# KarelPeeters/kZero

Measured on AMD Instinct MI355X. Metric: self-play NN evals/sec (node), Chess 20x256 ResNet b=256, 1/2/4/8 GPU, higher is better.
Workload: dtype f16; 1 GPU; chess-20x256 attention head, executor batch 256; engines_per_gpu=1, parallelism=dp1 (no collective)

## Files before the change

kzero_amd/csrc/kz_tower.hip:

```cpp
#include <cstdlib>
#include <type_traits>
#include <vector>

#include "kz_kernels.hpp"
#include "kz_launch.hpp"

namespace kz {

typedef _Float16 h16;
typedef h16 h16x8 __attribute__((ext_vector_type(8)));
typedef h16 h16x4 __attribute__((ext_vector_type(4)));
typedef float f32x4 __attribute__((ext_vector_type(4)));

namespace {

#include "kz_decode_dev.hpp"
#include "kz_encode_dev.hpp"

constexpr int C = 256;
constexpr int RS = C * 2 + 16;
constexpr int URS = 3 * C * 2 + 16;
constexpr int KSTEPS = 72;
constexpr int HEAD_KSTEPS = 5 * 8;
constexpr int POLICY = 1880, LOGIT_LD = 96;
constexpr int TOWER_PF_MAX = 8;

struct TowerDev {
    const h16 *x0;
    const uint4 *w_stem, *w_tower;
    const float *bias, *post_scale, *post_shift;
    h16 *y;
    int cin_p, batch, depth;
    PackedBoards in;
    const float *sh_w0, *sh_b0, *sh_w1, *sh_b1, *sh_w2, *sh_b2;
    const int32_t *att_idx;
    float *scalars, *policy;
    int *nonfinite_flag;
    int epoch;
    DecodeDev dec;
};

template <int I, int N, class F>
__device__ __forceinline__ void static_for(F &&f) {
    if constexpr (I < N) {
        f(std::integral_constant<int, I>{});
        static_for<I + 1, N>(f);
    }
}

template <int NB>
struct Layout {
    static constexpr int M = NB * 64;
    static constexpr int MT = M / 16;
    static constexpr bool LINE_TILES = NB == 2;
    static constexpr int BPAD = LINE_TILES ? 128 : 0;
    static constexpr int BOARD = 64 * RS + BPAD;
    static constexpr int TS = LINE_TILES ? 8 * RS : 16 * RS;
    static constexpr int IMG = NB * BOARD;
    static constexpr int X_OFF = 0;
    static constexpr int Y_OFF = IMG;
    static constexpr int Z_OFF = 2 * IMG;
    static_assert(Z_OFF % 256 == 0, "zero rows keep the slot pattern of the image rows");
    static constexpr int S_OFF = Z_OFF + 16 * RS;
    static constexpr int TOWER_BYTES = S_OFF + M * 64;
    static constexpr int U_OFF = Z_OFF;
    static constexpr int ACT_OFF = U_OFF + 16 * URS;
    static constexpr int HID_OFF = ACT_OFF + NB * 256 * 4;
    static constexpr int HEADS_BYTES = HID_OFF + NB * 32 * 4;
    static constexpr int LOG_OFF = Y_OFF;
    static constexpr int BYTES = TOWER_BYTES > HEADS_BYTES ? TOWER_BYTES : HEADS_BYTES;
    static_assert(NB * 64 * LOGIT_LD * 4 <= IMG, "logits fit the Y region");
    static constexpr int row_off(int b, int p) { return b * BOARD + p * RS; }
    static_assert(BYTES <= 160 * 1024, "LDS budget");
};

constexpr int SG_VALU = 0x2, SG_SALU = 0x4, SG_MFMA = 0x8, SG_VMEM_READ = 0x20, SG_DS_READ = 0x100;

template <int NB, bool HEADS, int PF, bool WIDE = false, bool PREV = false>
__global__ __launch_bounds__(256, 1) void kz_tower_resident(TowerDev a) {
    using L = Layout<NB>;
    constexpr int M = L::M, MT = L::MT;
    static_assert(PF <= TOWER_PF_MAX, "the refills past the end of the stream must land in its padding");
    extern __shared__ __attribute__((aligned(16))) unsigned char lds[];

    const int tid = threadIdx.x;
    const int wave = __builtin_amdgcn_readfirstlane(tid >> 6);
    const int lane = tid & 63;
    const int fr = lane & 15, kq = lane >> 4;
    const int board0 = blockIdx.x * NB;
    const int layers = 2 * a.depth;
    const int total_ksteps = layers * KSTEPS + (HEADS ? HEAD_KSTEPS : 0);
    const int bias_rows = layers + (HEADS ? 5 : 0);

    const uint4 *wp = a.w_tower + wave * 256 + lane;
    auto wload_prev = [&](int gk, int nt) __attribute__((always_inline)) { return wp[(size_t)gk * 1024 + nt * 64]; };
    typedef const __attribute__((address_space(1))) unsigned char *gptr;
    gptr wk = (gptr)a.w_tower + wave * 4096;
    const unsigned wlane = lane * 16;
    auto wload = [&](gptr k, int nt) __attribute__((always_inline)) {
        typedef unsigned u32x4 __attribute__((ext_vector_type(4)));
        return __builtin_bit_cast(uint4, *reinterpret_cast<const __attribute__((address_space(1))) u32x4 *>(k + wlane + nt * 1024));
    };
    uint4 wreg[PF][4];
#pragma unroll
    for (int s = 0; s < PF; s++) {
        const int g = s < total_ksteps ? s : total_ksteps - 1;
#pragma unroll
        for (int nt = 0; nt < 4; nt++) wreg[s][nt] = PREV ? wload_prev(g, nt) : wload(wk + s * 16384, nt);
    }
    wk += PF * 16384;
    int g = 0;
    auto ring_take = [&](int stage, h16x8 (&af)[4]) __attribute__((always_inline)) {
#pragma unroll
        for (int nt = 0; nt < 4; nt++) af[nt] = *reinterpret_cast<const h16x8 *>(&wreg[stage][nt]);
#ifndef KZ_TW_NO_WLOAD
        if constexpr (PREV) {
            const int gn = g + PF < total_ksteps ? g + PF : total_ksteps - 1;
#pragma unroll
            for (int nt = 0; nt < 4; nt++) wreg[stage][nt] = wload_prev(gn, nt);
        } else {
#pragma unroll
            for (int nt = 0; nt < 4; nt++) wreg[stage][nt] = wload(wk, nt);
        }
#endif
        wk += 16384;
        if constexpr (!PREV) asm("" : "+s"(wk));
    };

    const int sc = WIDE ? a.cin_p >> 5 : 1;
    const int stem_off = WIDE ? L::Y_OFF : L::S_OFF, srow = 64 * sc, spieces = 4 * sc;
    for (int id = tid; id < 16 * RS / 16; id += 256)
        *reinterpret_cast<uint4 *>(lds + L::Z_OFF + id * 16) = make_uint4(0, 0, 0, 0);
    for (int id = tid; id < M * spieces; id += 256) {
        const int row = WIDE ? id / spieces : id >> 2, c = id - row * spieces;
        const int board = board0 + (row >> 6);
        uint4 v = make_uint4(0, 0, 0, 0);
        if (board < a.batch) {
            if (a.in.bits) {
                h16x8 e;
#pragma unroll
                for (int j = 0; j < 8; j++) e[j] = (h16)encoded_plane(a.in, board, c * 8 + j, row & 63, 64);
                v = *reinterpret_cast<const uint4 *>(&e);
            } else {
                v = *reinterpret_cast<const uint4 *>(a.x0 + ((size_t)board0 * 64 + row) * a.cin_p + c * 8);
            }
        }
        *reinterpret_cast<uint4 *>(lds + stem_off + row * srow + c * 16) = v;
    }
    __syncthreads();

    f32x4 acc[4][MT];
    f32x4 bias_next[4];
    auto fetch_bias = [&](int row) __attribute__((always_inline)) {
        const int l = row <= bias_rows ? row : bias_rows;
#pragma unroll
        for (int nt = 0; nt < 4; nt++)
            bias_next[nt] = *reinterpret_cast<const f32x4 *>(a.bias + l * C + wave * 64 + nt * 16 + kq * 4);
    };
    auto init_acc = [&]() __attribute__((always_inline)) {
#pragma unroll
        for (int nt = 0; nt < 4; nt++)
#pragma unroll
            for (int mt = 0; mt < MT; mt++) acc[nt][mt] = bias_next[nt];
    };
    f32x4 post_s[4], post_t[4];
#pragma unroll
    for (int nt = 0; nt < 4; nt++) {
        post_s[nt] = f32x4{1.f, 1.f, 1.f, 1.f};
        post_t[nt] = f32x4{0.f, 0.f, 0.f, 0.f};
    }

    auto relu4 = [](f32x4 v) {
        typedef int i32x4 __attribute__((ext_vector_type(4)));
        i32x4 b = __builtin_bit_cast(i32x4, v);
#pragma unroll
        for (int j = 0; j < 4; j++) b[j] = b[j] > 0 ? b[j] : 0;
        return __builtin_bit_cast(f32x4, b);
    };
    auto to_h4 = [](f32x4 v) { return h16x4{(h16)v[0], (h16)v[1], (h16)v[2], (h16)v[3]}; };

    const int lane_row = L::LINE_TILES ? (fr >> 3) * L::BOARD + (fr & 7) * RS : fr * RS;
    const int epi_base = lane_row + (wave * 64 + kq * 4) * 2;
    auto epilogue = [&](int dst_off, auto relu, auto residual, auto post) __attribute__((always_inline)) {
#pragma unroll
        for (int nt = 0; nt < 4; nt++) {
            h16x4 rx[MT];
            if constexpr (decltype(residual)::value) {
#pragma unroll
                for (int mt = 0; mt < MT; mt++)
                    rx[mt] = *reinterpret_cast<const h16x4 *>(lds + L::X_OFF + epi_base + mt * L::TS + nt * 32);
            }
#pragma unroll
            for (int mt = 0; mt < MT; mt++) {
                const int off = epi_base + mt * L::TS + nt * 32;
                f32x4 v = acc[nt][mt];
                if constexpr (decltype(relu)::value) v = relu4(v);
                if constexpr (decltype(residual)::value) {
#pragma unroll
                    for (int j = 0; j < 4; j++) v[j] += (float)rx[mt][j];
                }
                if constexpr (decltype(post)::value) v = v * post_s[nt] + post_t[nt];
                *reinterpret_cast<h16x4 *>(lds + dst_off + off) = to_h4(v);
            }
        }
    };
    constexpr std::true_type YES{};
    constexpr std::false_type NO{};

    const bool x_is0 = (lane & 7) == 0, x_is7 = (lane & 7) == 7, yo_is0 = (lane & 8) == 0, yo_is1 = !yo_is0;
    auto tap_ok = [&](int mt, int dy, int dx) __attribute__((always_inline)) {
        const bool kill_x = (dx < 0 && x_is0) || (dx > 0 && x_is7);
        if constexpr (L::LINE_TILES) return !(kill_x || (dy < 0 && mt == 0) || (dy > 0 && mt == MT - 1));
        else return !(kill_x || ((mt & 3) == 0 && dy < 0 && yo_is0) || ((mt & 3) == 3 && dy > 0 && yo_is1));
    };

    fetch_bias(0);
    init_acc();
    fetch_bias(1);
    for (int ks = 0; ks < 9 * sc; ks++) {
        const int tap = WIDE ? ks / sc : ks, chunk = ks - tap * sc;
        const int dy = tap / 3 - 1, dx = tap % 3 - 1;
        h16x8 af[4];
#pragma unroll
        for (int nt = 0; nt < 4; nt++) {
            const uint4 t = a.w_stem[((ks * 4 + wave) * 4 + nt) * 64 + lane];
            af[nt] = *reinterpret_cast<const h16x8 *>(&t);
        }
#pragma unroll
        for (int mt = 0; mt < MT; mt++) {
            const bool ok = tap_ok(mt, dy, dx);
            const int p = L::LINE_TILES ? (fr >> 3) * 64 + mt * 8 + (fr & 7) : mt * 16 + fr;
            const int off = ok ? stem_off + (p + dy * 8 + dx) * srow + chunk * 64 + kq * 16 : L::Z_OFF + kq * 16;
            const h16x8 bf = *reinterpret_cast<const h16x8 *>(lds + off);
#pragma unroll
            for (int nt = 0; nt < 4; nt++)
                acc[nt][mt] = __builtin_amdgcn_mfma_f32_16x16x32_f16(af[nt], bf, acc[nt][mt], 0, 0, 0);
        }
    }
    epilogue(L::X_OFF, NO, NO, NO);
    __syncthreads();

    const int kq_off = 256 * (kq & 1) + 128 * (kq >> 1);
    const int frag_base = lane_row + kq_off;
    auto tap_rows = [&](int dy, int dx, int src_off, int (&T)[MT]) __attribute__((always_inline)) {
        const int shifted = frag_base + src_off + (dy * 8 + dx) * RS;
        const int zrow = L::Z_OFF + ((fr + dy * 8 + dx) & 15) * RS + kq_off;
        const int zrow_odd = L::LINE_TILES ? L::Z_OFF + ((fr + dy * 8 + dx + 8) & 15) * RS + kq_off : zrow;
        if constexpr (PREV) {
#pragma unroll
            for (int mt = 0; mt < MT; mt++) T[mt] = tap_ok(mt, dy, dx) ? shifted + mt * L::TS : ((mt & 1) ? zrow_odd : zrow);
        } else {
            int z0 = zrow, z1 = zrow_odd;
            asm("" : "+v"(z0), "+v"(z1));
            const bool kill_x = ((dx < 0) & x_is0) | ((dx > 0) & x_is7);
#pragma unroll
            for (int mt = 0; mt < MT; mt++) {
                bool kill = kill_x;
                if constexpr (!L::LINE_TILES) kill = kill_x | (((mt & 3) == 0) & (dy < 0) & yo_is0) | (((mt & 3) == 3) & (dy > 0) & yo_is1);
                T[mt] = kill ? ((mt & 1) ? z1 : z0) : shifted + mt * L::TS;
            }
        }
    };

    h16x8 bf[2][MT];
    constexpr auto tile_lo = [](int dy) { return L::LINE_TILES && dy < 0 ? 1 : 0; };
    constexpr auto tile_hi = [](int dy) { return L::LINE_TILES && dy > 0 ? MT - 1 : MT; };

    auto conv_plain = [&](auto ndy_tag, int src_off, int dx_lo, int dx_hi) __attribute__((always_inline)) {
        constexpr int NDY = decltype(ndy_tag)::value, DY0 = NDY == 3 ? -1 : 0;
        int T[NDY][MT], Tn[NDY][MT];
#pragma unroll
        for (int i = 0; i < NDY; i++) tap_rows(DY0 + i, dx_lo, src_off, T[i]);
#pragma unroll
        for (int mt = tile_lo(DY0); mt < tile_hi(DY0); mt++) bf[0][mt] = *reinterpret_cast<const h16x8 *>(lds + T[0][mt]);
#pragma nounroll
        for (int dx = dx_lo; dx < dx_hi; dx++) {
#pragma unroll
            for (int i = 0; i < NDY; i++) tap_rows(DY0 + i, dx + 1 < dx_hi ? dx + 1 : dx, src_off, Tn[i]);
            static_for<0, 8 * NDY>([&](auto s_tag) __attribute__((always_inline)) {
                constexpr int s = decltype(s_tag)::value, ch = s / NDY, i = s % NDY, dy = DY0 + i;
                constexpr int stage = s & (PF - 1), cur = s & 1, nxt = cur ^ 1;
                constexpr int lo = tile_lo(dy), hi = tile_hi(dy), nt_ = hi - lo;
                constexpr int in_ = (i + 1) % NDY, chn = i + 1 < NDY ? ch : ch + 1;
                constexpr int lon = tile_lo(DY0 + in_), hin = tile_hi(DY0 + in_), nr = hin - lon;
#ifndef KZ_TW_NO_DSREAD
#pragma unroll
                for (int mt = 0; mt < MT; mt++) {
                    if (mt >= lon && mt < hin)
                        bf[nxt][mt] = *reinterpret_cast<const h16x8 *>(lds + (chn < 8 ? T[in_][mt] + chn * 16 : Tn[in_][mt]));
                }
#endif
                h16x8 af[4];
                ring_take(stage, af);
#pragma unroll
                for (int nt = 0; nt < 4; nt++)
#pragma unroll
                    for (int mt = 0; mt < MT; mt++)
                        if (mt >= lo && mt < hi)
                            acc[nt][mt] = __builtin_amdgcn_mfma_f32_16x16x32_f16(af[nt], bf[cur][mt], acc[nt][mt], 0, 0, 0);
#pragma unroll
                for (int j = 0; j < 4; j++) {
                    __builtin_amdgcn_sched_group_barrier(SG_MFMA, 1, 0);
                    __builtin_amdgcn_sched_group_barrier(SG_VMEM_READ, 1, 0);
                }
#pragma unroll
                for (int j = 0; j < MT; j++) {
                    if (j < nr) {
                        __builtin_amdgcn_sched_group_barrier(SG_MFMA, 1, 0);
                        __builtin_amdgcn_sched_group_barrier(SG_DS_READ, 1, 0);
                    }
                }
                constexpr int n_free = 4 * nt_ - (nr + 4), n_alu = PREV || s != 0 ? 0 : n_free < 20 ? n_free : 20;
#pragma unroll
                for (int j = 0; j < 20; j++) {
                    if (j < n_alu) {
                        __builtin_amdgcn_sched_group_barrier(SG_MFMA, 1, 0);
                        __builtin_amdgcn_sched_group_barrier(SG_VALU | SG_SALU, 2, 0);
                    }
                }
                __builtin_amdgcn_sched_group_barrier(SG_MFMA, n_free - n_alu, 0);
                __builtin_amdgcn_sched_barrier(0);
                g++;
            });
#pragma unroll
            for (int i = 0; i < NDY; i++)
#pragma unroll
                for (int mt = 0; mt < MT; mt++) T[i][mt] = Tn[i][mt];
        }
    };

    auto conv_3x3_lines = [&](int src_off) __attribute__((always_inline)) {
        static_assert(!L::LINE_TILES || MT == 8, "one tile per board line");
        int T[MT], Tn[MT];
        tap_rows(0, -1, src_off, T);
#pragma unroll
        for (int mt = 0; mt < MT; mt++) bf[0][mt] = *reinterpret_cast<const h16x8 *>(lds + T[mt]);
#pragma nounroll
        for (int dx = -1; dx < 2; dx++) {
            tap_rows(0, dx < 1 ? dx + 1 : dx, src_off, Tn);
            static_for<0, 8>([&](auto ch_tag) __attribute__((always_inline)) {
                constexpr int ch = decltype(ch_tag)::value, cur = ch & 1, nxt = cur ^ 1;
#ifndef KZ_TW_NO_DSREAD
#pragma unroll
                for (int mt = 0; mt < MT; mt++)
                    bf[nxt][mt] = *reinterpret_cast<const h16x8 *>(lds + (ch < 7 ? T[mt] + (ch + 1) * 16 : Tn[mt]));
#endif
                static_for<0, 3>([&](auto i_tag) __attribute__((always_inline)) {
                    constexpr int i = decltype(i_tag)::value, dy = i - 1, stage = (ch * 3 + i) & (PF - 1);
                    constexpr int lo = tile_lo(dy), hi = tile_hi(dy), nt_ = hi - lo;
                    h16x8 af[4];
                    ring_take(stage, af);
#pragma unroll
                    for (int nt = 0; nt < 4; nt++)
#pragma unroll
                        for (int mt = 0; mt < MT; mt++)
                            if (mt >= lo && mt < hi)
                                acc[nt][mt] = __builtin_amdgcn_mfma_f32_16x16x32_f16(af[nt], bf[cur][mt + dy], acc[nt][mt], 0, 0, 0);
#pragma unroll
                    for (int j = 0; j < 4; j++) {
                        __builtin_amdgcn_sched_group_barrier(SG_MFMA, 1, 0);
                        __builtin_amdgcn_sched_group_barrier(SG_VMEM_READ, 1, 0);
                    }
                    constexpr int nr = i == 0 ? MT : 0;
#pragma unroll
                    for (int j = 0; j < MT; j++) {
                        if (j < nr) {
                            __builtin_amdgcn_sched_group_barrier(SG_MFMA, 1, 0);
                            __builtin_amdgcn_sched_group_barrier(SG_DS_READ, 1, 0);
                        }
                    }
                    constexpr int n_free = 4 * nt_ - (nr + 4), n_alu = ch == 0 && i == 0 ? n_free : 0;
#pragma unroll
                    for (int j = 0; j < 4 * MT; j++) {
                        if (j < n_alu) {
                            __builtin_amdgcn_sched_group_barrier(SG_MFMA, 1, 0);
                            __builtin_amdgcn_sched_group_barrier(SG_VALU | SG_SALU, 2, 0);
                        }
                    }
                    __builtin_amdgcn_sched_group_barrier(SG_MFMA, n_free - n_alu, 0);
                    __builtin_amdgcn_sched_barrier(0);
                    g++;
                });
            });
#pragma unroll
            for (int mt = 0; mt < MT; mt++) T[mt] = Tn[mt];
        }
    };
    constexpr std::integral_constant<int, 3> THREE_ROWS{};
    constexpr std::integral_constant<int, 1> ONE_ROW{};
    auto conv_3x3 = [&](int src_off) __attribute__((always_inline)) {
        if constexpr (L::LINE_TILES && !PREV) conv_3x3_lines(src_off);
        else conv_plain(THREE_ROWS, src_off, -1, 2);
    };
    auto conv_1x1 = [&](int src_off) __attribute__((always_inline)) { conv_plain(ONE_ROW, src_off, 0, 1); };

    for (int layer = 1; layer <= layers; layer++) {
        const bool is_b = (layer & 1) == 0;
        init_acc();
        fetch_bias(layer + 1);
        if (layer == layers) {
#pragma unroll
            for (int nt = 0; nt < 4; nt++) {
                const int oc = wave * 64 + nt * 16 + kq * 4;
                post_s[nt] = *reinterpret_cast<const f32x4 *>(a.post_scale + oc);
                post_t[nt] = *reinterpret_cast<const f32x4 *>(a.post_shift + oc);
            }
        }
        conv_3x3(is_b ? L::Y_OFF : L::X_OFF);
        if (!is_b) epilogue(L::Y_OFF, YES, NO, NO);
        else if (layer != layers) epilogue(L::X_OFF, YES, YES, NO);
        else epilogue(L::X_OFF, YES, YES, YES);
        __syncthreads();
    }

    if constexpr (!HEADS) {
        for (int id = tid; id < M * 32; id += 256) {
            const int p = id >> 5, c16 = id & 31;
            const int board = board0 + (p >> 6);
            if (board < a.batch) {
                const uint4 v = *reinterpret_cast<const uint4 *>(lds + L::X_OFF + L::row_off(p >> 6, p & 63) + c16 * 16);
                *reinterpret_cast<uint4 *>(a.y + ((size_t)board0 * 64 + p) * C + c16 * 8) = v;
            }
        }
    } else {
        {
            float *act = reinterpret_cast<float *>(lds + L::ACT_OFF);
            for (int o = tid; o < NB * 256; o += 256) {
                const int b = o >> 8, c4 = (o >> 6) & 3, p = o & 63;
                const unsigned char *row = lds + L::X_OFF + L::row_off(b, p);
                const float *w = a.sh_w0 + c4 * C;
                float s = a.sh_b0[c4];
#pragma unroll 4
                for (int i = 0; i < C; i += 8) {
                    const h16x8 xv = *reinterpret_cast<const h16x8 *>(row + i * 2);
                    const f32x4 w0 = *reinterpret_cast<const f32x4 *>(w + i), w1 = *reinterpret_cast<const f32x4 *>(w + i + 4);
#pragma unroll
                    for (int j = 0; j < 4; j++) s += (float)xv[j] * w0[j] + (float)xv[4 + j] * w1[j];
                }
                if (!(fabsf(s) <= 3.0e38f) && a.nonfinite_flag && board0 + b < a.batch) {
                    *reinterpret_cast<volatile int *>(a.nonfinite_flag) = a.epoch;
                    raise_nonfinite_board(a.nonfinite_flag, a.epoch, board0 + b);
                }
                act[o] = fmaxf(s, 0.0f);
            }
        }

        {
            const int tb = L::X_OFF + L::row_off(NB == 2 ? fr >> 3 : 0, 56 + (fr & 7)) + kq_off;
            for (int s = 0; s < 3; s++) {
                f32x4 ua[4];
#pragma unroll
                for (int nt = 0; nt < 4; nt++) ua[nt] = bias_next[nt];
                fetch_bias(layers + 2 + s);
#pragma unroll
                for (int ch = 0; ch < 8; ch++) {
                    const h16x8 bf = *reinterpret_cast<const h16x8 *>(lds + tb + ch * 16);
                    h16x8 af[4];
                    ring_take(ch & (PF - 1), af);
#pragma unroll
                    for (int nt = 0; nt < 4; nt++)
                        ua[nt] = __builtin_amdgcn_mfma_f32_16x16x32_f16(af[nt], bf, ua[nt], 0, 0, 0);
                    g++;
                }
                if (NB == 2 || fr < 8) {
#pragma unroll
                    for (int nt = 0; nt < 4; nt++)
                        *reinterpret_cast<h16x4 *>(lds + L::U_OFF + fr * URS + (256 * s + wave * 64 + nt * 16 + kq * 4) * 2) =
                            to_h4(ua[nt]);
                }
            }
        }

        init_acc();
        fetch_bias(layers + 5);
        conv_1x1(L::X_OFF);
        epilogue(L::Y_OFF, NO, NO, NO);

        init_acc();
        conv_1x1(L::X_OFF);
        __syncthreads();
        epilogue(L::X_OFF, NO, NO, NO);
        __syncthreads();

        {
            const float *act = reinterpret_cast<const float *>(lds + L::ACT_OFF);
            float *hid = reinterpret_cast<float *>(lds + L::HID_OFF);
            if (tid < NB * 128) {
                const int pair = tid >> 2, part = tid & 3, b = pair >> 5, j = pair & 31;
                const float *w = a.sh_w1 + j * 256 + part * 64;
                const float *x = act + b * 256 + part * 64;
                float s = 0.0f;
#pragma unroll 4
                for (int i = 0; i < 64; i += 4) {
                    const f32x4 wv = *reinterpret_cast<const f32x4 *>(w + i), xv = *reinterpret_cast<const f32x4 *>(x + i);
                    s += wv[0] * xv[0] + wv[1] * xv[1] + wv[2] * xv[2] + wv[3] * xv[3];
                }
                s += __shfl_xor(s, 1, 64);
                s += __shfl_xor(s, 2, 64);
                if (part == 0) hid[b * 32 + j] = fmaxf(s + a.sh_b1[j], 0.0f);
            }
        }

        constexpr int IT = NB == 2 ? 2 : 1;
        const int hb = NB == 2 ? wave >> 1 : 0;
        const int it0 = NB == 2 ? (wave & 1) * 2 : wave;
        f32x4 la[IT][6];
        {
            int ja[6], ia[IT];
#pragma unroll
            for (int jt = 0; jt < 4; jt++) ja[jt] = L::X_OFF + L::row_off(hb, jt * 16 + fr) + kq_off;
            ja[4] = L::U_OFF + (hb * 8 + (fr & 7)) * URS + (fr >> 3) * 512 + kq_off;
            ja[5] = L::U_OFF + (hb * 8 + (fr & 7)) * URS + 2 * 512 + kq_off;
#pragma unroll
            for (int ii = 0; ii < IT; ii++) ia[ii] = L::Y_OFF + L::row_off(hb, (it0 + ii) * 16 + fr) + kq_off;
#pragma unroll
            for (int ii = 0; ii < IT; ii++)
#pragma unroll
                for (int jt = 0; jt < 6; jt++) la[ii][jt] = f32x4{0.f, 0.f, 0.f, 0.f};
#pragma unroll
            for (int ch = 0; ch < 8; ch++) {
                h16x8 qa[6], qb[IT];
#pragma unroll
                for (int jt = 0; jt < 6; jt++) qa[jt] = *reinterpret_cast<const h16x8 *>(lds + ja[jt] + ch * 16);
#pragma unroll
                for (int ii = 0; ii < IT; ii++) qb[ii] = *reinterpret_cast<const h16x8 *>(lds + ia[ii] + ch * 16);
#pragma unroll
                for (int ii = 0; ii < IT; ii++)
#pragma unroll
                    for (int jt = 0; jt < 6; jt++)
                        la[ii][jt] = __builtin_amdgcn_mfma_f32_16x16x32_f16(qa[jt], qb[ii], la[ii][jt], 0, 0, 0);
            }
        }
        __syncthreads();
        {
            const float inv = 1.0f / sqrtf((float)C);
#pragma unroll
            for (int ii = 0; ii < IT; ii++)
#pragma unroll
                for (int jt = 0; jt < 6; jt++) {
                    const int i = (it0 + ii) * 16 + fr, j = jt * 16 + kq * 4;
                    *reinterpret_cast<f32x4 *>(lds + L::LOG_OFF + ((hb * 64 + i) * LOGIT_LD + j) * 4) = la[ii][jt] * inv;
                }
        }
        const bool decode = a.dec.move_offsets != nullptr;
        float *raw = reinterpret_cast<float *>(lds + L::ACT_OFF);
        if (tid < NB * 5) {
            const int b = tid / 5, k = tid % 5;
            const float *hid = reinterpret_cast<const float *>(lds + L::HID_OFF) + b * 32;
            float s = a.sh_b2[k];
            for (int i = 0; i < 32; i++) s += a.sh_w2[k * 32 + i] * hid[i];
            if (decode) raw[b * 8 + k] = s;
            else if (board0 + b < a.batch) a.scalars[(size_t)(board0 + b) * 5 + k] = s;
        }
        __syncthreads();
        if (decode) {
            if (wave < NB && board0 + wave < a.batch) {
                const float *lg = reinterpret_cast<const float *>(lds + L::LOG_OFF) + wave * 64 * LOGIT_LD;
                float *stage = reinterpret_cast<float *>(lds + L::X_OFF + L::row_off(wave, 0));
                decode_board_wave(a.dec, board0 + wave, lane, raw + wave * 8, stage, 64 * RS / 4,
                                  [&](int idx) { return lg[a.att_idx[idx]]; });
            }
        } else {
            for (int b = 0; b < NB; b++) {
                if (board0 + b >= a.batch) break;
                const float *lg = reinterpret_cast<const float *>(lds + L::LOG_OFF) + b * 64 * LOGIT_LD;
                float *pol = a.policy + (size_t)(board0 + b) * POLICY;
                for (int k = tid; k < POLICY; k += 256) pol[k] = lg[a.att_idx[k]];
            }
        }
    }
}

#ifndef KZ_PF_NB1
#define KZ_PF_NB1 4
#endif
#ifndef KZ_PF_NB2
#define KZ_PF_NB2 4
#endif
constexpr int PF_NB1 = KZ_PF_NB1, PF_NB2 = KZ_PF_NB2;

void pack_1x1(const float *w, uint16_t *dst) {
    static const int kq_base[4] = {0, 128, 64, 192};
    for (int chunk = 0; chunk < 8; chunk++)
        for (int wave = 0; wave < 4; wave++)
            for (int nt = 0; nt < 4; nt++)
                for (int lane = 0; lane < 64; lane++)
                    for (int j = 0; j < 8; j++) {
                        const int oc = 64 * wave + 16 * nt + (lane & 15);
                        const int ch = 8 * chunk + kq_base[lane >> 4] + j;
                        const _Float16 hv = (_Float16)w[(size_t)oc * 256 + ch];
                        uint16_t bits;
                        __builtin_memcpy(&bits, &hv, 2);
                        dst[((((size_t)chunk * 4 + wave) * 4 + nt) * 64 + lane) * 8 + j] = bits;
                    }
}

}

bool tower_resident_supported(int dtype, int h, int w, int channels, int depth, int c_in) {
    return dtype == 1 && h == 8 && w == 8 && channels == C && depth >= 1 && c_in >= 1 && c_in <= 224;
}

bool tower_heads_supported(int policy_kind, int query_channels, int policy_len, int sh_channels, int sh_size) {
    return policy_kind == 2 && query_channels == C && policy_len == POLICY && sh_channels == 4 && sh_size == 32;
}

size_t tower_packed_weight_elems(int cin_p, int depth) {
    return (size_t)9 * C * cin_p + (size_t)2 * depth * 9 * C * C;
}

size_t tower_heads_weight_elems() { return (size_t)HEAD_KSTEPS * 16 * 1024 / 2; }

size_t tower_weight_pad_elems() { return (size_t)TOWER_PF_MAX * 16 * 1024 / 2; }

void tower_pack_weights(const float *oihw, int cout, int cin, int cin_p, uint16_t *dst, bool tap_major) {
    const int nchunk = cin_p / 32;
    const bool rows_inner = cin_p == 256 && !tap_major;
    static const int kq_base[4] = {0, 128, 64, 192};
    for (int tap = 0; tap < 9; tap++)
        for (int chunk = 0; chunk < nchunk; chunk++) {
            const size_t kstep = rows_inner ? ((size_t)(tap % 3) * 8 + chunk) * 3 + tap / 3 : (size_t)tap * nchunk + chunk;
            for (int wave = 0; wave < 4; wave++)
                for (int nt = 0; nt < 4; nt++)
                    for (int lane = 0; lane < 64; lane++)
                        for (int j = 0; j < 8; j++) {
                            const int oc = 64 * wave + 16 * nt + (lane & 15);
                            const int kq = lane >> 4;
                            const int ch = cin_p == 256 ? 8 * chunk + kq_base[kq] + j : 32 * chunk + 8 * kq + j;
                            float v = 0.0f;
                            if (oc < cout && ch < cin) v = oihw[((size_t)oc * cin + ch) * 9 + tap];
                            const _Float16 hv = (_Float16)v;
                            uint16_t bits;
                            __builtin_memcpy(&bits, &hv, 2);
                            dst[(((kstep * 4 + wave) * 4 + nt) * 64 + lane) * 8 + j] = bits;
                        }
        }
}

void tower_pack_heads(const float *w_bulk , const float *b_bulk, const float *w_under ,
                      const float *b_under, uint16_t *dst, float *bias5) {
    const size_t pass = (size_t)8 * 16 * 1024 / 2;
    std::vector<float> tmp((size_t)256 * 256);
    for (int s = 0; s < 3; s++) {
        for (int q = 0; q < 256; q++) {
            for (int c = 0; c < 256; c++) tmp[(size_t)q * 256 + c] = w_under[(size_t)(3 * q + s) * 256 + c];
            bias5[s * 256 + q] = b_under[3 * q + s];
        }
        pack_1x1(tmp.data(), dst + pass * s);
    }
    pack_1x1(w_bulk, dst + pass * 3);
    pack_1x1(w_bulk + (size_t)256 * 256, dst + pass * 4);
    for (int q = 0; q < 256; q++) {
        bias5[3 * 256 + q] = b_bulk[q];
        bias5[4 * 256 + q] = b_bulk[256 + q];
    }
}

namespace {
template <auto Kernel>
void launch_instance(const TowerDev &d, int grid, int bytes, hipStream_t stream) {
    allow_dynamic_lds<Kernel>(bytes);
    Kernel<<<grid, 256, bytes, stream>>>(d);
}
}

void launch_tower_resident(const TowerArgs &t, hipStream_t stream) {
    TowerDev d{};
    d.x0 = static_cast<const h16 *>(t.x0);
    d.w_stem = static_cast<const uint4 *>(t.w_stem);
    d.w_tower = static_cast<const uint4 *>(t.w_tower);
    d.bias = t.bias;
    d.post_scale = t.post_scale;
    d.post_shift = t.post_shift;
    d.y = static_cast<h16 *>(t.y);
    d.cin_p = t.cin_p;
    d.batch = t.batch;
    d.depth = t.depth;
    d.in = t.in;
    d.sh_w0 = t.sh_w0; d.sh_b0 = t.sh_b0; d.sh_w1 = t.sh_w1; d.sh_b1 = t.sh_b1; d.sh_w2 = t.sh_w2; d.sh_b2 = t.sh_b2;
    d.att_idx = t.att_idx;
    d.scalars = t.scalars;
    d.policy = t.policy;
    d.nonfinite_flag = t.nonfinite_flag;
    d.epoch = t.epoch;
    d.dec = decode_dev(t.decode, t.fused_heads, POLICY);
    const bool heads = t.fused_heads;
#ifdef KZ_EXPERIMENTS
    if (t.prev) {
        const int grid = (t.batch + 1) / 2;
        if (t.cin_p > 32) {
            if (heads) launch_instance<kz_tower_resident<2, true, PF_NB2, true, true>>(d, grid, Layout<2>::BYTES, stream);
            else launch_instance<kz_tower_resident<2, false, PF_NB2, true, true>>(d, grid, Layout<2>::BYTES, stream);
        } else if (t.boards_per_wg == 1) {
            if (heads) launch_instance<kz_tower_resident<1, true, PF_NB1, false, true>>(d, t.batch, Layout<1>::BYTES, stream);
            else launch_instance<kz_tower_resident<1, false, PF_NB1, false, true>>(d, t.batch, Layout<1>::BYTES, stream);
        } else {
            if (heads) launch_instance<kz_tower_resident<2, true, PF_NB2, false, true>>(d, grid, Layout<2>::BYTES, stream);
            else launch_instance<kz_tower_resident<2, false, PF_NB2, false, true>>(d, grid, Layout<2>::BYTES, stream);
        }
        return;
    }
#endif
    if (t.cin_p > 32) {
        const int grid = (t.batch + 1) / 2;
        if (heads) launch_instance<kz_tower_resident<2, true, PF_NB2, true>>(d, grid, Layout<2>::BYTES, stream);
        else launch_instance<kz_tower_resident<2, false, PF_NB2, true>>(d, grid, Layout<2>::BYTES, stream);
    } else if (t.boards_per_wg == 1) {
        if (heads) launch_instance<kz_tower_resident<1, true, PF_NB1>>(d, t.batch, Layout<1>::BYTES, stream);
        else launch_instance<kz_tower_resident<1, false, PF_NB1>>(d, t.batch, Layout<1>::BYTES, stream);
    } else {
        const int grid = (t.batch + 1) / 2;
        if (heads) launch_instance<kz_tower_resident<2, true, PF_NB2>>(d, grid, Layout<2>::BYTES, stream);
        else launch_instance<kz_tower_resident<2, false, PF_NB2>>(d, grid, Layout<2>::BYTES, stream);
    }
}

}
```

Baseline: 539,100 evals/s.

## Seed accumulators from bias in first MFMA and stage post-affine in LDS

The first k-step of each conv now takes the bias registers as the MFMA accumulator input, so the separate init_acc copy disappears and the next layer's bias fetch moves into the loop after that first step. The final post-scale/shift vectors move from per-lane registers into an LDS slab. ReLU-only epilogues convert to f16 first and clamp with a packed integer max. Ring stage indices become modulo-PF with a per-pass offset, which allows non-power-of-two prefetch depths. The aim is to cut register pressure and VALU work around layer boundaries, at the cost of extra LDS and more complex scheduling.

```diff
diff --git a/kzero_amd/csrc/kz_tower.hip b/kzero_amd/csrc/kz_tower.hip
--- a/kzero_amd/csrc/kz_tower.hip
+++ b/kzero_amd/csrc/kz_tower.hip
@@ -62,7 +62,8 @@
     static constexpr int Z_OFF = 2 * IMG;
     static_assert(Z_OFF % 256 == 0, "zero rows keep the slot pattern of the image rows");
     static constexpr int S_OFF = Z_OFF + 16 * RS;
-    static constexpr int TOWER_BYTES = S_OFF + M * 64;
+    static constexpr int POST_OFF = S_OFF + M * 64;
+    static constexpr int TOWER_BYTES = POST_OFF + 2 * 256 * 4;
     static constexpr int U_OFF = Z_OFF;
     static constexpr int ACT_OFF = U_OFF + 16 * URS;
     static constexpr int HID_OFF = ACT_OFF + NB * 256 * 4;
@@ -81,6 +82,8 @@
     using L = Layout<NB>;
     constexpr int M = L::M, MT = L::MT;
     static_assert(PF <= TOWER_PF_MAX, "the refills past the end of the stream must land in its padding");
+    static_assert(24 % PF == 0 && KSTEPS % PF == 0, "a k-step's ring stage is its index within the pass (+ the pass's offset) % PF");
+    static_assert(!PREV || PF == 4, "the reference instances keep the ring they were measured with");
     extern __shared__ __attribute__((aligned(16))) unsigned char lds[];
 
     const int tid = threadIdx.x;
@@ -178,10 +181,21 @@
         return __builtin_bit_cast(f32x4, b);
     };
     auto to_h4 = [](f32x4 v) { return h16x4{(h16)v[0], (h16)v[1], (h16)v[2], (h16)v[3]}; };
+    auto to_h4_relu = [](f32x4 v) {
+        typedef float f32x2 __attribute__((ext_vector_type(2)));
+        typedef h16 h16x2 __attribute__((ext_vector_type(2)));
+        typedef short i16x2 __attribute__((ext_vector_type(2)));
+        const i16x2 zero{0, 0};
+        const i16x2 lo = __builtin_elementwise_max(__builtin_bit_cast(i16x2, __builtin_convertvector(f32x2{v[0], v[1]}, h16x2)), zero);
+        const i16x2 hi = __builtin_elementwise_max(__builtin_bit_cast(i16x2, __builtin_convertvector(f32x2{v[2], v[3]}, h16x2)), zero);
+        return uint2{__builtin_bit_cast(unsigned, lo), __builtin_bit_cast(unsigned, hi)};
+    };
 
     const int lane_row = L::LINE_TILES ? (fr >> 3) * L::BOARD + (fr & 7) * RS : fr * RS;
-    const int epi_base = lane_row + (wave * 64 + kq * 4) * 2;
+    const int epi_base_lane = lane_row + (wave * 64 + kq * 4) * 2;
     auto epilogue = [&](int dst_off, auto relu, auto residual, auto post) __attribute__((always_inline)) {
+        int epi_base = epi_base_lane;
+        if constexpr (!PREV) asm volatile("" : "+v"(epi_base));
 #pragma unroll
         for (int nt = 0; nt < 4; nt++) {
             h16x4 rx[MT];
@@ -194,13 +208,25 @@
             for (int mt = 0; mt < MT; mt++) {
                 const int off = epi_base + mt * L::TS + nt * 32;
                 f32x4 v = acc[nt][mt];
-                if constexpr (decltype(relu)::value) v = relu4(v);
-                if constexpr (decltype(residual)::value) {
-#pragma unroll
-                    for (int j = 0; j < 4; j++) v[j] += (float)rx[mt][j];
-                }
-                if constexpr (decltype(post)::value) v = v * post_s[nt] + post_t[nt];
-                *reinterpret_cast<h16x4 *>(lds + dst_off + off) = to_h4(v);
+                if constexpr (!PREV) asm volatile("" : "+v"(v));
+                if constexpr (decltype(relu)::value && !decltype(residual)::value && !decltype(post)::value && !PREV) {
+                    *reinterpret_cast<uint2 *>(lds + dst_off + off) = to_h4_relu(v);
+                } else {
+                    if constexpr (decltype(relu)::value) v = relu4(v);
+                    if constexpr (decltype(residual)::value) {
+#pragma unroll
+                        for (int j = 0; j < 4; j++) v[j] += (float)rx[mt][j];
+                    }
+                    if constexpr (decltype(post)::value) {
+                        if constexpr (PREV) {
+                            v = v * post_s[nt] + post_t[nt];
+                        } else {
+                            const float *ps = reinterpret_cast<const float *>(lds + L::POST_OFF) + wave * 64 + nt * 16 + kq * 4;
+                            v = v * *reinterpret_cast<const f32x4 *>(ps) + *reinterpret_cast<const f32x4 *>(ps + C);
+                        }
+                    }
+                    *reinterpret_cast<h16x4 *>(lds + dst_off + off) = to_h4(v);
+                }
             }
         }
     };
@@ -217,6 +243,11 @@
     fetch_bias(0);
     init_acc();
     fetch_bias(1);
+    float post_lane[2] = {0.f, 0.f};
+    if constexpr (!PREV) {
+        post_lane[0] = a.post_scale[tid];
+        post_lane[1] = a.post_shift[tid];
+    }
     for (int ks = 0; ks < 9 * sc; ks++) {
         const int tap = WIDE ? ks / sc : ks, chunk = ks - tap * sc;
         const int dy = tap / 3 - 1, dx = tap % 3 - 1;
@@ -236,6 +267,10 @@
             for (int nt = 0; nt < 4; nt++)
                 acc[nt][mt] = __builtin_amdgcn_mfma_f32_16x16x32_f16(af[nt], bf, acc[nt][mt], 0, 0, 0);
         }
+    }
+    if constexpr (!PREV) {
+        reinterpret_cast<float *>(lds + L::POST_OFF)[tid] = post_lane[0];
+        reinterpret_cast<float *>(lds + L::POST_OFF)[C + tid] = post_lane[1];
     }
     epilogue(L::X_OFF, NO, NO, NO);
     __syncthreads();
@@ -266,20 +301,26 @@
     constexpr auto tile_lo = [](int dy) { return L::LINE_TILES && dy < 0 ? 1 : 0; };
     constexpr auto tile_hi = [](int dy) { return L::LINE_TILES && dy > 0 ? MT - 1 : MT; };
 
-    auto conv_plain = [&](auto ndy_tag, int src_off, int dx_lo, int dx_hi) __attribute__((always_inline)) {
-        constexpr int NDY = decltype(ndy_tag)::value, DY0 = NDY == 3 ? -1 : 0;
+    auto conv_plain = [&](auto ndy_tag, auto stage0_tag, int src_off, int dx_lo, int dx_hi, auto fetch_next) __attribute__((always_inline)) {
+        constexpr int NDY = decltype(ndy_tag)::value, DY0 = NDY == 3 ? -1 : 0, STAGE0 = decltype(stage0_tag)::value;
+        static_assert(PREV || (tile_lo(DY0) == 0 && tile_hi(DY0) == MT), "the first k-step starts every accumulator");
         int T[NDY][MT], Tn[NDY][MT];
+        if constexpr (PREV) {
+            init_acc();
+            fetch_next();
+        }
 #pragma unroll
         for (int i = 0; i < NDY; i++) tap_rows(DY0 + i, dx_lo, src_off, T[i]);
 #pragma unroll
         for (int mt = tile_lo(DY0); mt < tile_hi(DY0); mt++) bf[0][mt] = *reinterpret_cast<const h16x8 *>(lds + T[0][mt]);
-#pragma nounroll
-        for (int dx = dx_lo; dx < dx_hi; dx++) {
+        auto dx_body = [&](auto first_tag, int dx) __attribute__((always_inline)) {
+            constexpr bool FIRST = decltype(first_tag)::value;
 #pragma unroll
             for (int i = 0; i < NDY; i++) tap_rows(DY0 + i, dx + 1 < dx_hi ? dx + 1 : dx, src_off, Tn[i]);
             static_for<0, 8 * NDY>([&](auto s_tag) __attribute__((always_inline)) {
                 constexpr int s = decltype(s_tag)::value, ch = s / NDY, i = s % NDY, dy = DY0 + i;
-                constexpr int stage = s & (PF - 1), cur = s & 1, nxt = cur ^ 1;
+                constexpr int stage = (STAGE0 + s) % PF, cur = s & 1, nxt = cur ^ 1;
+                constexpr bool from_bias = FIRST && s == 0;
                 constexpr int lo = tile_lo(dy), hi = tile_hi(dy), nt_ = hi - lo;
                 constexpr int in_ = (i + 1) % NDY, chn = i + 1 < NDY ? ch : ch + 1;
                 constexpr int lon = tile_lo(DY0 + in_), hin = tile_hi(DY0 + in_), nr = hin - lon;
@@ -297,7 +338,7 @@
 #pragma unroll
                     for (int mt = 0; mt < MT; mt++)
                         if (mt >= lo && mt < hi)
-                            acc[nt][mt] = __builtin_amdgcn_mfma_f32_16x16x32_f16(af[nt], bf[cur][mt], acc[nt][mt], 0, 0, 0);
+                            acc[nt][mt] = __builtin_amdgcn_mfma_f32_16x16x32_f16(af[nt], bf[cur][mt], from_bias ? bias_next[nt] : acc[nt][mt], 0, 0, 0);
 #pragma unroll
                 for (int j = 0; j < 4; j++) {
                     __builtin_amdgcn_sched_group_barrier(SG_MFMA, 1, 0);
@@ -321,22 +362,31 @@
                 __builtin_amdgcn_sched_group_barrier(SG_MFMA, n_free - n_alu, 0);
                 __builtin_amdgcn_sched_barrier(0);
                 g++;
+                if constexpr (from_bias) fetch_next();
             });
 #pragma unroll
             for (int i = 0; i < NDY; i++)
 #pragma unroll
                 for (int mt = 0; mt < MT; mt++) T[i][mt] = Tn[i][mt];
-        }
-    };
-
-    auto conv_3x3_lines = [&](int src_off) __attribute__((always_inline)) {
+        };
+        if constexpr (PREV) {
+#pragma nounroll
+            for (int dx = dx_lo; dx < dx_hi; dx++) dx_body(NO, dx);
+        } else {
+            dx_body(YES, dx_lo);
+#pragma nounroll
+            for (int dx = dx_lo + 1; dx < dx_hi; dx++) dx_body(NO, dx);
+        }
+    };
+
+    auto conv_3x3_lines = [&](int src_off, auto fetch_next) __attribute__((always_inline)) {
         static_assert(!L::LINE_TILES || MT == 8, "one tile per board line");
         int T[MT], Tn[MT];
         tap_rows(0, -1, src_off, T);
 #pragma unroll
         for (int mt = 0; mt < MT; mt++) bf[0][mt] = *reinterpret_cast<const h16x8 *>(lds + T[mt]);
-#pragma nounroll
-        for (int dx = -1; dx < 2; dx++) {
+        auto dx_body = [&](auto first_tag, int dx) __attribute__((always_inline)) {
+            constexpr bool FIRST = decltype(first_tag)::value;
             tap_rows(0, dx < 1 ? dx + 1 : dx, src_off, Tn);
             static_for<0, 8>([&](auto ch_tag) __attribute__((always_inline)) {
                 constexpr int ch = decltype(ch_tag)::value, cur = ch & 1, nxt = cur ^ 1;
@@ -346,7 +396,7 @@
                     bf[nxt][mt] = *reinterpret_cast<const h16x8 *>(lds + (ch < 7 ? T[mt] + (ch + 1) * 16 : Tn[mt]));
 #endif
                 static_for<0, 3>([&](auto i_tag) __attribute__((always_inline)) {
-                    constexpr int i = decltype(i_tag)::value, dy = i - 1, stage = (ch * 3 + i) & (PF - 1);
+                    constexpr int i = decltype(i_tag)::value, dy = i - 1, stage = (ch * 3 + i) % PF;
                     constexpr int lo = tile_lo(dy), hi = tile_hi(dy), nt_ = hi - lo;
                     h16x8 af[4];
                     ring_take(stage, af);
@@ -354,8 +404,10 @@
                     for (int nt = 0; nt < 4; nt++)
 #pragma unroll
                         for (int mt = 0; mt < MT; mt++)
-                            if (mt >= lo && mt < hi)
-                                acc[nt][mt] = __builtin_amdgcn_mfma_f32_16x16x32_f16(af[nt], bf[cur][mt + dy], acc[nt][mt], 0, 0, 0);
+                            if (mt >= lo && mt < hi) {
+                                const bool from_bias = FIRST && ch == 0 && (i == 0 || (i == 1 && mt == 0));
+                                acc[nt][mt] = __builtin_amdgcn_mfma_f32_16x16x32_f16(af[nt], bf[cur][mt + dy], from_bias ? bias_next[nt] : acc[nt][mt], 0, 0, 0);
+                            }
 #pragma unroll
                     for (int j = 0; j < 4; j++) {
                         __builtin_amdgcn_sched_group_barrier(SG_MFMA, 1, 0);
@@ -381,24 +433,28 @@
                     __builtin_amdgcn_sched_barrier(0);
                     g++;
                 });
+                if constexpr (FIRST && ch == 0) fetch_next();
             });
 #pragma unroll
             for (int mt = 0; mt < MT; mt++) T[mt] = Tn[mt];
-        }
+        };
+        dx_body(YES, -1);
+#pragma nounroll
+        for (int dx = 0; dx < 2; dx++) dx_body(NO, dx);
     };
     constexpr std::integral_constant<int, 3> THREE_ROWS{};
     constexpr std::integral_constant<int, 1> ONE_ROW{};
-    auto conv_3x3 = [&](int src_off) __attribute__((always_inline)) {
-        if constexpr (L::LINE_TILES && !PREV) conv_3x3_lines(src_off);
-        else conv_plain(THREE_ROWS, src_off, -1, 2);
-    };
-    auto conv_1x1 = [&](int src_off) __attribute__((always_inline)) { conv_plain(ONE_ROW, src_off, 0, 1); };
+    auto conv_3x3 = [&](int src_off, auto fetch_next) __attribute__((always_inline)) {
+        if constexpr (L::LINE_TILES && !PREV) conv_3x3_lines(src_off, fetch_next);
+        else conv_plain(THREE_ROWS, std::integral_constant<int, 0>{}, src_off, -1, 2, fetch_next);
+    };
+    auto conv_1x1 = [&](auto pass_tag, int src_off, auto fetch_next) __attribute__((always_inline)) {
+        conv_plain(ONE_ROW, std::integral_constant<int, decltype(pass_tag)::value * 8 % PF>{}, src_off, 0, 1, fetch_next);
+    };
 
     for (int layer = 1; layer <= layers; layer++) {
         const bool is_b = (layer & 1) == 0;
-        init_acc();
-        fetch_bias(layer + 1);
-        if (layer == layers) {
+        if (PREV && layer == layers) {
 #pragma unroll
             for (int nt = 0; nt < 4; nt++) {
                 const int oc = wave * 64 + nt * 16 + kq * 4;
@@ -406,7 +462,7 @@
                 post_t[nt] = *reinterpret_cast<const f32x4 *>(a.post_shift + oc);
             }
         }
-        conv_3x3(is_b ? L::Y_OFF : L::X_OFF);
+        conv_3x3(is_b ? L::Y_OFF : L::X_OFF, [&]() __attribute__((always_inline)) { fetch_bias(layer + 1); });
         if (!is_b) epilogue(L::Y_OFF, YES, NO, NO);
         else if (layer != layers) epilogue(L::X_OFF, YES, YES, NO);
         else epilogue(L::X_OFF, YES, YES, YES);
@@ -447,7 +503,8 @@
 
         {
             const int tb = L::X_OFF + L::row_off(NB == 2 ? fr >> 3 : 0, 56 + (fr & 7)) + kq_off;
-            for (int s = 0; s < 3; s++) {
+            static_for<0, 3>([&](auto s_tag) __attribute__((always_inline)) {
+                constexpr int s = decltype(s_tag)::value;
                 f32x4 ua[4];
 #pragma unroll
                 for (int nt = 0; nt < 4; nt++) ua[nt] = bias_next[nt];
@@ -456,7 +513,7 @@
                 for (int ch = 0; ch < 8; ch++) {
                     const h16x8 bf = *reinterpret_cast<const h16x8 *>(lds + tb + ch * 16);
                     h16x8 af[4];
-                    ring_take(ch & (PF - 1), af);
+                    ring_take((8 * s + ch) % PF, af);
 #pragma unroll
                     for (int nt = 0; nt < 4; nt++)
                         ua[nt] = __builtin_amdgcn_mfma_f32_16x16x32_f16(af[nt], bf, ua[nt], 0, 0, 0);
@@ -468,16 +525,13 @@
                         *reinterpret_cast<h16x4 *>(lds + L::U_OFF + fr * URS + (256 * s + wave * 64 + nt * 16 + kq * 4) * 2) =
                             to_h4(ua[nt]);
                 }
-            }
-        }
-
-        init_acc();
-        fetch_bias(layers + 5);
-        conv_1x1(L::X_OFF);
+            });
+        }
+
+        conv_1x1(std::integral_constant<int, 3>{}, L::X_OFF, [&]() __attribute__((always_inline)) { fetch_bias(layers + 5); });
         epilogue(L::Y_OFF, NO, NO, NO);
 
-        init_acc();
-        conv_1x1(L::X_OFF);
+        conv_1x1(std::integral_constant<int, 4>{}, L::X_OFF, []() {});
         __syncthreads();
         epilogue(L::X_OFF, NO, NO, NO);
         __syncthreads();
@@ -689,14 +743,14 @@
     if (t.prev) {
         const int grid = (t.batch + 1) / 2;
         if (t.cin_p > 32) {
-            if (heads) launch_instance<kz_tower_resident<2, true, PF_NB2, true, true>>(d, grid, Layout<2>::BYTES, stream);
-            else launch_instance<kz_tower_resident<2, false, PF_NB2, true, true>>(d, grid, Layout<2>::BYTES, stream);
+            if (heads) launch_instance<kz_tower_resident<2, true, 4, true, true>>(d, grid, Layout<2>::BYTES, stream);
+            else launch_instance<kz_tower_resident<2, false, 4, true, true>>(d, grid, Layout<2>::BYTES, stream);
         } else if (t.boards_per_wg == 1) {
-            if (heads) launch_instance<kz_tower_resident<1, true, PF_NB1, false, true>>(d, t.batch, Layout<1>::BYTES, stream);
-            else launch_instance<kz_tower_resident<1, false, PF_NB1, false, true>>(d, t.batch, Layout<1>::BYTES, stream);
+            if (heads) launch_instance<kz_tower_resident<1, true, 4, false, true>>(d, t.batch, Layout<1>::BYTES, stream);
+            else launch_instance<kz_tower_resident<1, false, 4, false, true>>(d, t.batch, Layout<1>::BYTES, stream);
         } else {
-            if (heads) launch_instance<kz_tower_resident<2, true, PF_NB2, false, true>>(d, grid, Layout<2>::BYTES, stream);
-            else launch_instance<kz_tower_resident<2, false, PF_NB2, false, true>>(d, grid, Layout<2>::BYTES, stream);
+            if (heads) launch_instance<kz_tower_resident<2, true, 4, false, true>>(d, grid, Layout<2>::BYTES, stream);
+            else launch_instance<kz_tower_resident<2, false, 4, false, true>>(d, grid, Layout<2>::BYTES, stream);
         }
         return;
     }
```

Result: no change. 542,800 evals/s (median of 6 runs) (+0.7%).
